# Ewenwan/ORB_SLAM2_SSD_Semantic

Measured on AMD Instinct MI355X. Metric: ORB extract+match frames/sec on 640x480 TUM RGB-D; bit-exact kp/desc, higher is better.
Workload: dtype u8

## Files before the change

orb_slam2_ssd_semantic_amd/csrc/orbfe_fast_body_u.inc:

```
    uint32_t *lflag = s_cf + wv * cf_words;
    for (int i = lane; i < cf_words; i += 64) lflag[i] = 0u;
    const OrbLane ld = lanes[(int64_t)t * 64 + lane];
    const int level = __builtin_amdgcn_readfirstlane((int)(ld.flags >> 8));
    const OrbLevel &L = plan->lv[level];
    int pitch;
    const uint8_t *src = level_ptr(fs, L, level, b, &pitch);
    uint2 *slist = skeys + (int64_t)b * plan->keys_per_frame + L.key_off;
    int32_t *scnt = scount + (b * plan->nlevels + level) * ORBFE_NK_STRIDE;
    uint32_t *cflag = cflags + (int64_t)(b * plan->nlevels + level) * cf_words;
    const int ini_th = plan->ini_th;
    uint2 *sbuf = s_buf[wv];
    int nbuf = 0;
    int st_rows = 0, st_arc = 0, st_nms = 0;
    const int key_cap = L.key_cap;
    const int ix0 = ORBFE_EDGE, iy0 = ORBFE_EDGE, ix1 = L.ix1;
    const int wcell = L.wcell, hcell = L.hcell;
    const int x = ld.x;
    const int ys = ld.ys;
    const int nrows = __builtin_amdgcn_readfirstlane((int)ld.nrows);
    const int nsteps = nrows + 7;
    const int tz = max(plan->min_th, 1);

    int ccj[4], mj[4];
    {
        const int r0 = max(x - ix0, 0);
        int c = r0 / wcell, m = r0 - c * wcell;
#pragma unroll
        for (int j = 0; j < 4; ++j) {
            if (j > 0 && x + j - ix0 >= 1) {
                ++m;
                if (m == wcell) { m = 0; ++c; }
            }
            ccj[j] = c;
            mj[j] = m;
        }
    }
    int inside = 0, lvalid = 0, rvalid = 0;
#pragma unroll
    for (int j = 0; j < 4; ++j) {
        const int xx = x + j;
        if (xx >= ix0 && xx < ix1) {
            const int m = mj[j];
            inside |= 1 << j;
            if (m != 0) lvalid |= 1 << j;
            if (m != wcell - 1 && xx + 1 < ix1) rvalid |= 1 << j;
        }
    }
    auto halves = [](int bits, int j) -> uint32_t {
        return (((bits >> j) & 1) ? 0xFFFFu : 0u) | (((bits >> (j + 1)) & 1) ? 0xFFFF0000u : 0u);
    };
    const uint32_t in01 = halves(inside, 0), in23 = halves(inside, 2);
    const uint32_t lv01 = halves(lvalid, 0), lv23 = halves(lvalid, 2);
    const uint32_t rv01 = halves(rvalid, 0), rv23 = halves(rvalid, 2);
    const bool split01 = (inside & 3) == 3 && !(lvalid & 2), split23 = (inside & 12) == 12 && !(lvalid & 8);
    const bool wave_split = orb_ballot(split01 || split23) != 0ull;
    const bool out_lane = !(ld.flags & 1) && inside != 0;
    const unsigned long long bout = orb_ballot(out_lane);
    uint32_t ordx[4];
    {
        const uint32_t row_part = (uint32_t)(((ys - iy0) / hcell) * L.ncc) << 12;
#pragma unroll
        for (int j = 0; j < 4; ++j) ordx[j] = row_part + (((uint32_t)ccj[j] << 12) | (uint32_t)mj[j]);
    }
    int rmod = 0;
    uint32_t ordy = 0u;
    const uint32_t ord_wrap = ((uint32_t)L.ncc << 12) - ((uint32_t)hcell << 6);
    const uint32_t tzz = (uint32_t)tz * 0x00010001u;
    const uint32_t resp0 = (uint32_t)(tz - 1);
    const uint32_t key00 = (uint32_t)(x - ORBFE_MINB) + ((uint32_t)(ys - 7 - ORBFE_MINB) << 12);

    uint32_t R[8][FM_NE], Raw[2][3];
    uint32_t S01[8], S23[8];
#pragma unroll
    for (int k = 0; k < 8; ++k) {
        S01[k] = S23[k] = 0u;
#pragma unroll
        for (int i = 0; i < FM_NE; ++i) R[k][i] = 0u;
    }
    const __amdgpu_buffer_rsrc_t rsrc = __builtin_amdgcn_make_buffer_rsrc((void *)src, 0, -1, 0x00020000);
    const int voff = (ys - 3) * pitch + x - 4;
    typedef uint32_t fmu_v3 __attribute__((ext_vector_type(3)));
    auto fetch = [&](int s, uint32_t (&dst3)[3]) {
        const fmu_v3 w = __builtin_amdgcn_raw_buffer_load_b96(rsrc, voff, s * pitch, 0);
        dst3[0] = w.x;
        dst3[1] = w.y;
        dst3[2] = w.z;
    };
    fetch(0, Raw[0]);

    for (int s0 = 0; s0 < nsteps; s0 += 8) {
#pragma unroll
        for (int k = 0; k < 8; ++k) {
            const int s = s0 + k;
            if (s >= nsteps) break;
            const bool have_row = s < nrows + 6;
            fetch(s + 1, Raw[(k + 1) % 2]);
            fast_unpack_row(Raw[k % 2], R[k]);
            if (s < 6) continue;
            if (have_row) {
                const uint32_t(&rm3)[FM_NE] = R[(k + 2) % 8];
                const uint32_t(&rm2)[FM_NE] = R[(k + 3) % 8];
                const uint32_t(&rm1)[FM_NE] = R[(k + 4) % 8];
                const uint32_t(&r0)[FM_NE] = R[(k + 5) % 8];
                const uint32_t(&rp1)[FM_NE] = R[(k + 6) % 8];
                const uint32_t(&rp2)[FM_NE] = R[(k + 7) % 8];
                const uint32_t(&rp3)[FM_NE] = R[k];
                bool arcs = true;
                if (SPARSE) {
                    const uint32_t p = (fast_compass_pair<0>(rm3, r0, rp3, tzz) & in01) |
                                       (fast_compass_pair<2>(rm3, r0, rp3, tzz) & in23);
                    arcs = orb_ballot(p != 0u) != 0ull;
#ifdef ORBFE_DEVELOPER
                    if (plan->dbg == 60) arcs = false;
#endif
                    if (fstat) { st_rows++; st_arc += arcs ? 0 : 1; }
                }
                if (arcs) {
                    S01[k] = fast_strength_pair<0>(rm3, rm2, rm1, r0, rp1, rp2, rp3, tzz) & in01;
                    S23[k] = fast_strength_pair<2>(rm3, rm2, rm1, r0, rp1, rp2, rp3, tzz) & in23;
                } else {
                    S01[k] = S23[k] = 0u;
                }
            }
            if (s < 7) continue;
            const int ku = (k + 6) % 8, km = (k + 7) % 8;
            const bool up_ok = rmod != 0;
            const bool dn_ok = rmod != hcell - 1 && have_row;
            const uint32_t ord_row = ordy;
            {
                const bool wrap = rmod == hcell - 1;
                rmod = wrap ? 0 : rmod + 1;
                ordy += wrap ? 64u + ord_wrap : 64u;
            }
            if (SPARSE) {
                if (orb_ballot((S01[km] | S23[km]) != 0u) == 0ull) {
                    if (fstat) st_nms++;
                    continue;
                }
            }
            const uint32_t u01 = up_ok ? S01[ku] : 0u, u23 = up_ok ? S23[ku] : 0u;
            const uint32_t d01 = dn_ok ? S01[k] : 0u, d23 = dn_ok ? S23[k] : 0u;
            const uint32_t m01 = S01[km], m23 = S23[km];
            const uint32_t v01 = pk_max_u16(u01, d01), v23 = pk_max_u16(u23, d23);
            const uint32_t c01 = pk_max_u16(v01, m01), c23 = pk_max_u16(v23, m23);
            const uint32_t cL = (uint32_t)__builtin_amdgcn_update_dpp(0, (int)c23, 0x138, 0xF, 0xF, true);
            const uint32_t cR = (uint32_t)__builtin_amdgcn_update_dpp(0, (int)c01, 0x130, 0xF, 0xF, true);
            const uint32_t l01 = __builtin_amdgcn_alignbit(c01, cL, 16) & lv01;
            const uint32_t x12 = __builtin_amdgcn_alignbit(c23, c01, 16);
            const uint32_t r23 = __builtin_amdgcn_alignbit(cR, c23, 16) & rv23;
            const uint32_t n01 = pk_max3(l01, x12 & rv01, v01);
            const uint32_t n23 = pk_max3(x12 & lv23, r23, v23);
            const uint32_t g01 = pk_subsat_u16(m01, n01), g23 = pk_subsat_u16(m23, n23);
            const unsigned long long b01 = orb_ballot(g01 != 0u) & bout, b23 = orb_ballot(g23 != 0u) & bout;
            const bool has01 = out_lane && g01 != 0u, has23 = out_lane && g23 != 0u;
            if (b01 | b23) {
                const uint32_t keyrow = key00 + ((uint32_t)s << 12);
                const int p01 = __popcll(b01);
                if (has01) {
                    const bool hi = g01 > 0xFFFFu;
                    const uint32_t a = hi ? m01 >> 16 : m01 & 0xFFFFu;
                    sbuf[nbuf + lanes_below(b01)] = make_uint2(keyrow + (hi ? 1u : 0u) + ((a + resp0) << 24),
                                                               ord_row + (hi ? ordx[1] : ordx[0]));
                }
                if (has23) {
                    const bool hi = g23 > 0xFFFFu;
                    const uint32_t a = hi ? m23 >> 16 : m23 & 0xFFFFu;
                    sbuf[nbuf + p01 + lanes_below(b23)] = make_uint2(keyrow + (hi ? 3u : 2u) + ((a + resp0) << 24),
                                                                     ord_row + (hi ? ordx[3] : ordx[2]));
                }
                nbuf += p01 + __popcll(b23);
                if (wave_split) {
                    const uint32_t gs = split01 ? g01 : (split23 ? g23 : 0u);
                    const bool dbl = out_lane && (gs & 0xFFFFu) != 0u && gs > 0xFFFFu;
                    const unsigned long long bd = orb_ballot(dbl);
                    if (bd) {
                        if (dbl) {
                            const uint32_t a = (split23 ? m23 : m01) & 0xFFFFu;
                            sbuf[nbuf + lanes_below(bd)] = make_uint2(keyrow + (split23 ? 2u : 0u) + ((a + resp0) << 24),
                                                                      ord_row + (split23 ? ordx[2] : ordx[0]));
                        }
                        nbuf += __popcll(bd);
                    }
                }
                if (nbuf > FM_BUF - FM_ROW_MAX) {
                    fm_flush(slist, scnt, sbuf, nbuf, key_cap, lane, lflag, ini_th);
                    nbuf = 0;
                }
            }
        }
    }
    if (nbuf > 0) fm_flush(slist, scnt, sbuf, nbuf, key_cap, lane, lflag, ini_th);
    __builtin_amdgcn_fence(__ATOMIC_ACQ_REL, "workgroup");
    for (int i = lane; i < cf_words; i += 64) {
        const uint32_t v = lflag[i];
        if (v) atomicOr(&cflag[i], v);
    }
    if (SPARSE && fstat && lane == 0) {
        atomicAdd(&fstat[0], (unsigned long long)st_rows);
        atomicAdd(&fstat[1], (unsigned long long)st_arc);
        atomicAdd(&fstat[2], (unsigned long long)st_nms);
    }
```

orb_slam2_ssd_semantic_amd/csrc/orbfe_kernels.hip:

```cpp
#include <stdio.h>
#include <stdlib.h>
#include <algorithm>

#include "orbfe_common.h"
#include "orbfe_kernels.h"
#include "orbfe_pattern.inc"

__constant__ signed char c_pattern[1024];
__constant__ int c_umax[16];

hipError_t orbk_upload_moment_weights(const int *umax16);

hipError_t orbk_upload_constants(const int *umax16)
{
    hipError_t e = hipMemcpyToSymbol(HIP_SYMBOL(c_pattern), orbfe_pattern31_host, 1024);
    if (e != hipSuccess) return e;
    e = hipMemcpyToSymbol(HIP_SYMBOL(c_umax), umax16, 16 * sizeof(int));
    if (e != hipSuccess) return e;
    return orbk_upload_moment_weights(umax16);
}

typedef _Float16 orb_h2 __attribute__((ext_vector_type(2)));
typedef short orb_s2 __attribute__((ext_vector_type(2)));
typedef unsigned short orb_u2 __attribute__((ext_vector_type(2)));
// ... 316 lines not shown
            uint32_t Hs[4];
            hsum(raw[(k + 1) % 4], Hs);
            const bool emit = lane_ok && d < yend && (int)(short)cur.y + 1 == r0 + s;
            const uint32_t b0 = cur.x & 0xFFFFu, b1 = cur.x >> 16;
            uint32_t pa[4], pb[4];
#pragma unroll
            for (int j = 0; j < 4; ++j) {
                pa[j] = __umul24(b0, Hp[j]);
                pb[j] = __umul24(b1, Hs[j]) + 0x20000u;
            }
            uint32_t t01, t23;
            asm("v_add_u32_sdwa %0, %1, %2 dst_sel:DWORD dst_unused:UNUSED_PAD src0_sel:WORD_1 src1_sel:WORD_1" : "=v"(t01) : "v"(pa[0]), "v"(pb[0]));
            asm("v_add_u32_sdwa %0, %1, %2 dst_sel:WORD_1 dst_unused:UNUSED_PRESERVE src0_sel:WORD_1 src1_sel:WORD_1" : "+v"(t01) : "v"(pa[1]), "v"(pb[1]));
            asm("v_add_u32_sdwa %0, %1, %2 dst_sel:DWORD dst_unused:UNUSED_PAD src0_sel:WORD_1 src1_sel:WORD_1" : "=v"(t23) : "v"(pa[2]), "v"(pb[2]));
            asm("v_add_u32_sdwa %0, %1, %2 dst_sel:WORD_1 dst_unused:UNUSED_PRESERVE src0_sel:WORD_1 src1_sel:WORD_1" : "+v"(t23) : "v"(pa[3]), "v"(pb[3]));
            const uint32_t q01 = __builtin_bit_cast(uint32_t, __builtin_bit_cast(orb_u2, t01) >> (orb_u2)(2));
            const uint32_t q23 = __builtin_bit_cast(uint32_t, __builtin_bit_cast(orb_u2, t23) >> (orb_u2)(2));
            if (emit) {
                *park = __builtin_amdgcn_perm(q23, q01, 0x06040200u);
                park += GX;
                d += 1;
            }
            cur = s_yt[min(d, yend) - by0];
#pragma unroll
            for (int j = 0; j < 4; ++j) Hp[j] = Hs[j];
        }
    }
    if (lane_ok && g0 + cg < ncol4) {
        uint32_t oofs = __umul24((uint32_t)y0, (uint32_t)a.dpitch) + (uint32_t)dx0;
        const int nrows = yend - y0;
        for (int i0 = 0; i0 < a.rb; i0 += 8) {
            uint32_t v[8];
#pragma unroll
            for (int i = 0; i < 8; ++i) v[i] = s_tile[(yl0 + min(i0 + i, a.rb - 1)) * GX + cg];
#pragma unroll
            for (int i = 0; i < 8; ++i)
                if (i0 + i < nrows) *(uint32_t *)(dst + (oofs + (uint32_t)(i0 + i) * (uint32_t)a.dpitch)) = v[i];
        }
    }
    __syncthreads();
    const int cx0 = p.cxs[tx], cx1 = p.cxs[tx + 1], cy0 = p.cys[ty], cy1 = p.cys[ty + 1];
    if (cx1 <= cx0 || cy1 <= cy0) return;
    const int gq0 = cx0 >> 2, ngc = ((cx1 - 1) >> 2) - gq0 + 1;
    const int nch = max(1, 256 / ngc);
    const int gi = (int)threadIdx.x % ngc, chn = (int)threadIdx.x / ngc;
    if (chn >= nch) return;
    const int nrowsC = cy1 - cy0, per = (nrowsC + nch - 1) / nch;
    const int ya = cy0 + chn * per, yb = min(ya + per, cy1);
    const uint8_t *T = (const uint8_t *)s_tile;
    const int tpitch = GX * 4, bx0 = g0 * 4;
    const int colmax = min(GX * 4, W - bx0) - 1, rowmax = min(trows, H - by0) - 1;
    uint8_t *dstC = p.dstC + (int64_t)b * a.dst_fstride;
    const int xg = (gq0 + gi) * 4;
    int c0i[4], c1i[4];
    uint32_t cc0[4], cc1[4];
    bool ok[4];
#pragma unroll
    for (int j = 0; j < 4; ++j) {
        const int x2 = xg + j;
        ok[j] = x2 >= cx0 && x2 < cx1;
        const OrbTab tt = p.xtabC[min(x2, p.cw - 1)];
        c0i[j] = min(max((int)tt.s - bx0, 0), colmax);
        c1i[j] = min(c0i[j] + 1, colmax);
        cc0[j] = (uint32_t)(uint16_t)tt.c0;
        cc1[j] = (uint32_t)(uint16_t)tt.c1;
    }
    const bool full = ok[0] && ok[1] && ok[2] && ok[3];
    OrbTab tyn = p.ytabC[min(ya, p.ch - 1)];
    for (int y2 = ya; y2 < yb; ++y2) {
        const OrbTab ty_ = tyn;
        tyn = p.ytabC[min(y2 + 1, p.ch - 1)];
        const int rr0 = (int)ty_.s - by0, rr1 = min(rr0 + 1, rowmax);
        const uint32_t b0 = (uint32_t)(uint16_t)ty_.c0, b1 = (uint32_t)(uint16_t)ty_.c1;
        const uint8_t *R0 = T + rr0 * tpitch, *R1 = T + rr1 * tpitch;
        uint32_t px[4];
#pragma unroll
        for (int j = 0; j < 4; ++j) {
            const uint32_t H0 = (R0[c0i[j]] * cc0[j] + R0[c1i[j]] * cc1[j]) >> 4, H1 = (R1[c0i[j]] * cc0[j] + R1[c1i[j]] * cc1[j]) >> 4;
            px[j] = ((((b0 * H0) >> 16) + ((b1 * H1) >> 16) + 2u) >> 2) & 0xFFu;
        }
        uint8_t *o = dstC + (__umul24((uint32_t)y2, (uint32_t)p.cpitch) + (uint32_t)xg);
        if (full) {
            *(uint32_t *)o = px[0] | (px[1] << 8) | (px[2] << 16) | (px[3] << 24);
        } else {
#pragma unroll
            for (int j = 0; j < 4; ++j)
                if (ok[j]) o[j] = (uint8_t)px[j];
        }
    }
}
#endif

__device__ __forceinline__ unsigned long long orb_ballot(bool p) { return __builtin_amdgcn_ballot_w64(p); }
__device__ __forceinline__ int min3i(int a, int b, int c) { return min(min(a, b), c); }
__device__ __forceinline__ int max3i(int a, int b, int c) { return max(max(a, b), c); }



__device__ __forceinline__ uint32_t pk_min3(uint32_t a, uint32_t b, uint32_t c)
{
    const orb_h2 x = __builtin_bit_cast(orb_h2, a), y = __builtin_bit_cast(orb_h2, b), z = __builtin_bit_cast(orb_h2, c);
    return __builtin_bit_cast(uint32_t, __builtin_elementwise_minimum(__builtin_elementwise_minimum(x, y), z));
}
__device__ __forceinline__ uint32_t pk_max3(uint32_t a, uint32_t b, uint32_t c)
{
    const orb_h2 x = __builtin_bit_cast(orb_h2, a), y = __builtin_bit_cast(orb_h2, b), z = __builtin_bit_cast(orb_h2, c);
    return __builtin_bit_cast(uint32_t, __builtin_elementwise_maximum(__builtin_elementwise_maximum(x, y), z));
}
__device__ __forceinline__ uint32_t pk_sub_i16(uint32_t a, uint32_t b)
{
    return __builtin_bit_cast(uint32_t, __builtin_bit_cast(orb_s2, a) - __builtin_bit_cast(orb_s2, b));
}
__device__ __forceinline__ uint32_t pk_max_i16(uint32_t a, uint32_t b)
{
    return __builtin_bit_cast(uint32_t, __builtin_elementwise_max(__builtin_bit_cast(orb_s2, a), __builtin_bit_cast(orb_s2, b)));
}
__device__ __forceinline__ uint32_t pk_sub_u16(uint32_t a, uint32_t b)
{
    return __builtin_bit_cast(uint32_t, __builtin_bit_cast(orb_u2, a) - __builtin_bit_cast(orb_u2, b));
}
__device__ __forceinline__ uint32_t pk_max_u16(uint32_t a, uint32_t b)
{
    return __builtin_bit_cast(uint32_t, __builtin_elementwise_max(__builtin_bit_cast(orb_u2, a), __builtin_bit_cast(orb_u2, b)));
}
__device__ __forceinline__ uint32_t pk_min_u16(uint32_t a, uint32_t b)
{
    return __builtin_bit_cast(uint32_t, __builtin_elementwise_min(__builtin_bit_cast(orb_u2, a), __builtin_bit_cast(orb_u2, b)));
}
__device__ __forceinline__ uint32_t pk_subsat_u16(uint32_t a, uint32_t b)
{
    return __builtin_bit_cast(uint32_t, __builtin_elementwise_sub_sat(__builtin_bit_cast(orb_u2, a), __builtin_bit_cast(orb_u2, b)));
}

template <int IDX>
__device__ __forceinline__ uint32_t rowpair(const uint32_t (&w)[3])
{
    static_assert(IDX >= 0 && IDX < 11, "window pair");
    if ((IDX & 3) < 3)
        return __builtin_amdgcn_perm(0u, w[IDX >> 2], 0x0c000c00u | ((uint32_t)((IDX & 3) + 1) << 16) | (uint32_t)(IDX & 3));
    return __builtin_amdgcn_perm(w[(IDX >> 2) + 1 > 2 ? 2 : (IDX >> 2) + 1], w[IDX >> 2], 0x0c040c03u);
}

#define FM_NE 9
__device__ __forceinline__ void fast_unpack_row(const uint32_t (&w)[3], uint32_t (&e)[FM_NE])
{
    e[0] = rowpair<1>(w);
    e[1] = rowpair<2>(w);
    e[2] = rowpair<3>(w);
    e[3] = rowpair<4>(w);
    e[4] = rowpair<5>(w);
    e[5] = rowpair<6>(w);
    e[6] = rowpair<7>(w);
    e[7] = rowpair<8>(w);
    e[8] = rowpair<9>(w);
}

template <int J>
__device__ __forceinline__ uint32_t fast_strength_pair(const uint32_t (&rm3)[FM_NE], const uint32_t (&rm2)[FM_NE],
                                                       const uint32_t (&rm1)[FM_NE], const uint32_t (&r0)[FM_NE],
                                                       const uint32_t (&rp1)[FM_NE], const uint32_t (&rp2)[FM_NE],
                                                       const uint32_t (&rp3)[FM_NE], uint32_t t)
{
    uint32_t c[16];
    c[0] = rp3[3 + J];
    c[1] = rp3[4 + J];
    c[2] = rp2[5 + J];
    c[3] = rp1[6 + J];
    c[4] = r0[6 + J];
    c[5] = rm1[6 + J];
    c[6] = rm2[5 + J];
    c[7] = rm3[4 + J];
    c[8] = rm3[3 + J];
    c[9] = rm3[2 + J];
    c[10] = rm2[1 + J];
    c[11] = rm1[0 + J];
    c[12] = r0[0 + J];
    c[13] = rp1[0 + J];
    c[14] = rp2[1 + J];
    c[15] = rp3[2 + J];
    const uint32_t v = r0[3 + J];
    uint32_t P[8], Q[8], ex[8], en[8];
#pragma unroll
    for (int i = 0; i < 8; ++i) {
        P[i] = pk_min_u16(c[2 * i + 1], c[(2 * i + 2) & 15]);
        Q[i] = pk_max_u16(c[2 * i + 1], c[(2 * i + 2) & 15]);
        ex[i] = pk_max_u16(c[2 * i], c[(2 * i + 9) & 15]);
        en[i] = pk_min_u16(c[2 * i], c[(2 * i + 9) & 15]);
    }
    uint32_t Wb[8], Wd[8];
#pragma unroll
    for (int i = 0; i < 8; i += 2) {
        const uint32_t ab = pk_min3(P[i], P[(i + 1) & 7], P[(i + 2) & 7]);
        const uint32_t ad = pk_max3(Q[i], Q[(i + 1) & 7], Q[(i + 2) & 7]);
        Wb[i] = pk_min3(ab, P[(i + 3) & 7], ex[i]);
        Wd[i] = pk_max3(ad, Q[(i + 3) & 7], en[i]);
        Wb[(i + 7) & 7] = pk_min3(P[(i + 7) & 7], ab, ex[(i + 7) & 7]);
        Wd[(i + 7) & 7] = pk_max3(Q[(i + 7) & 7], ad, en[(i + 7) & 7]);
    }
    const uint32_t maxmin = pk_max_u16(pk_max3(pk_max3(pk_max3(Wb[0], Wb[1], Wb[2]), Wb[3], Wb[4]), Wb[5], Wb[6]), Wb[7]);
    const uint32_t minmax = pk_min_u16(pk_min3(pk_min3(pk_min3(Wd[0], Wd[1], Wd[2]), Wd[3], Wd[4]), Wd[5], Wd[6]), Wd[7]);
    const uint32_t m = pk_max3(pk_subsat_u16(v, minmax), pk_subsat_u16(maxmin, v), t);
    return pk_sub_u16(m, t);
}

template <int J>
__device__ __forceinline__ uint32_t fast_compass_pair(const uint32_t (&rm3)[FM_NE], const uint32_t (&r0)[FM_NE],
                                                      const uint32_t (&rp3)[FM_NE], uint32_t t)
{
    const uint32_t c0 = rp3[3 + J], c8 = rm3[3 + J];
    const uint32_t c4 = r0[6 + J], c12 = r0[0 + J];
    const uint32_t v = r0[3 + J];
    const uint32_t mb = pk_min_u16(pk_max_u16(c0, c8), pk_max_u16(c4, c12));
    const uint32_t md = pk_max_u16(pk_min_u16(c0, c8), pk_min_u16(c4, c12));
    return pk_subsat_u16(pk_max_u16(pk_subsat_u16(mb, v), pk_subsat_u16(v, md)), t);
}

__device__ __forceinline__ uint32_t fast_strength_from(const uint32_t (&c)[16], uint32_t v, uint32_t t)
{
    uint32_t P[8], Q[8], ex[8], en[8];
#pragma unroll
    for (int i = 0; i < 8; ++i) {
        P[i] = pk_min_u16(c[2 * i + 1], c[(2 * i + 2) & 15]);
        Q[i] = pk_max_u16(c[2 * i + 1], c[(2 * i + 2) & 15]);
        ex[i] = pk_max_u16(c[2 * i], c[(2 * i + 9) & 15]);
        en[i] = pk_min_u16(c[2 * i], c[(2 * i + 9) & 15]);
    }
    uint32_t Wb[8], Wd[8];
#pragma unroll
    for (int i = 0; i < 8; i += 2) {
        const uint32_t ab = pk_min3(P[i], P[(i + 1) & 7], P[(i + 2) & 7]);
        const uint32_t ad = pk_max3(Q[i], Q[(i + 1) & 7], Q[(i + 2) & 7]);
        Wb[i] = pk_min3(ab, P[(i + 3) & 7], ex[i]);
        Wd[i] = pk_max3(ad, Q[(i + 3) & 7], en[i]);
        Wb[(i + 7) & 7] = pk_min3(P[(i + 7) & 7], ab, ex[(i + 7) & 7]);
        Wd[(i + 7) & 7] = pk_max3(Q[(i + 7) & 7], ad, en[(i + 7) & 7]);
    }
    const uint32_t maxmin = pk_max_u16(pk_max3(pk_max3(pk_max3(Wb[0], Wb[1], Wb[2]), Wb[3], Wb[4]), Wb[5], Wb[6]), Wb[7]);
    const uint32_t minmax = pk_min_u16(pk_min3(pk_min3(pk_min3(Wd[0], Wd[1], Wd[2]), Wd[3], Wd[4]), Wd[5], Wd[6]), Wd[7]);
    const uint32_t m = pk_max3(pk_subsat_u16(v, minmax), pk_subsat_u16(maxmin, v), t);
    return pk_sub_u16(m, t);
}

__device__ __forceinline__ int lanes_below(unsigned long long m)
{
    return __builtin_amdgcn_mbcnt_hi((uint32_t)(m >> 32), __builtin_amdgcn_mbcnt_lo((uint32_t)m, 0));
}

#define FM_BUF 384
#define FM_ROW_MAX 140

__device__ __forceinline__ void fm_flush(uint2 *slist, int32_t *scnt, const uint2 *sbuf, int nbuf, int key_cap, int lane,
                                         uint32_t *lflag, int ini)
{
    int base = 0;
    if (lane == 0) base = atomicAdd(scnt, nbuf);
    base = __shfl(base, 0, 64);
    for (int i = lane; i < nbuf; i += 64) {
        const uint2 e = sbuf[i];
        if (base + i < key_cap) slist[base + i] = e;
        if (orb_key_r(e.x) >= ini) {
            const uint32_t cell = e.y >> 12;
            atomicOr(&lflag[cell >> 5], 1u << (cell & 31));
        }
    }
}

#if defined(FM_WAVES_PER_EU)
#define FM_OCC __attribute__((amdgpu_waves_per_eu(FM_WAVES_PER_EU, FM_WAVES_PER_EU)))
#else
#define FM_OCC
#endif
#define FM_SHARED_DECLS                                                                                             \
    __shared__ uint2 s_buf[4][FM_BUF];                                                                              \
    extern __shared__ uint32_t s_cf[];
#ifdef FM_LDS_CONSTS
#define FM_LDS_DECLS                                                             \
    __shared__ uint4 s_lcm[4][64];                   \
    __shared__ uint2 s_lcr[4][64];                               \
    __shared__ uint4 s_lco[4][64];
#else
#define FM_LDS_DECLS
#endif

template <int SPARSE>
__global__ __launch_bounds__(256) FM_OCC void k_fast_map(const OrbPlan *__restrict__ plan, FrameSrc fs,
                                                  const OrbLane *__restrict__ lanes, int nwaves,
                                                  uint2 *__restrict__ skeys,
                                                  int32_t *__restrict__ scount,
                                                  uint32_t *__restrict__ cflags,
                                                  int32_t cf_words,
                                                  unsigned long long *__restrict__ fstat)
{
    FM_SHARED_DECLS
    FM_LDS_DECLS
    int b = blockIdx.y, bx = blockIdx.x;
    xcd_frame_remap(bx, b);
    const int lane = threadIdx.x & 63;
    const int wv = threadIdx.x >> 6;
    const int t = bx * (blockDim.x >> 6) + wv;
    if (t >= nwaves) return;
#include "orbfe_fast_body.inc"
}

template <int SPARSE>
__global__ __launch_bounds__(256) FM_OCC void k_fast_map_u(const OrbPlan *__restrict__ plan, FrameSrc fs,
                                                    const OrbLane *__restrict__ lanes, int nwaves,
                                                    uint2 *__restrict__ skeys, int32_t *__restrict__ scount,
                                                    uint32_t *__restrict__ cflags, int32_t cf_words,
                                                    unsigned long long *__restrict__ fstat)
{
    FM_SHARED_DECLS
    int b = blockIdx.y, bx = blockIdx.x;
    xcd_frame_remap(bx, b);
    const int lane = threadIdx.x & 63;
    const int wv = threadIdx.x >> 6;
    const int t = bx * (blockDim.x >> 6) + wv;
    if (t >= nwaves) return;
#include "orbfe_fast_body_u.inc"
}

#define FC_QCAP 128
#ifndef FC_LAG
#define FC_LAG 3
#endif
#define FC_PN (6 + FC_LAG)
#define FC_PW 66
#define FC_SEAMS 16
#define FC_BUF (128 + FC_SEAMS)
#ifndef FC_OCC
#define FC_OCC
#endif
static_assert(FC_LAG >= 1 && FC_LAG <= 3, "the strength-row ring (srow / snap, 4 slots) is re-used by the front half of step s + 4: the back half of step s must have read it, i.e. lag <= 3");
static_assert(FC_PN >= 6 + FC_LAG && FC_PN >= 7, "pixel ring: the first row of an item parked at step s is overwritten at step s - 6 + FC_PN");
__device__ __forceinline__ uint32_t fast_compass_from(uint32_t c0, uint32_t c8, uint32_t c4, uint32_t c12, uint32_t v, uint32_t t)
{
    const uint32_t mb = pk_min_u16(pk_max_u16(c0, c8), pk_max_u16(c4, c12));
    const uint32_t md = pk_max_u16(pk_min_u16(c0, c8), pk_min_u16(c4, c12));
    return pk_subsat_u16(pk_max_u16(pk_subsat_u16(mb, v), pk_subsat_u16(v, md)), t);
}
__global__ __launch_bounds__(256) FC_OCC void k_fast_map_c(const OrbPlan *__restrict__ plan, FrameSrc fs,
                                                    const OrbLane *__restrict__ lanes, int nwaves,
                                                    uint2 *__restrict__ skeys, int32_t *__restrict__ scount,
                                                    uint32_t *__restrict__ cflags, int32_t cf_words,
                                                    unsigned long long *__restrict__ fstat)
{
    __shared__ uint32_t s_pix[4][2 * FC_PN * FC_PW];
#ifdef FC_EXTRA_LDS
    __shared__ uint32_t s_fcpad[FC_EXTRA_LDS / 4];
    if (nwaves < 0) s_fcpad[threadIdx.x] = 1u;
    if (nwaves < -1) scount[0] = (int32_t)s_fcpad[threadIdx.x ^ 1];
#endif
    __shared__ uint32_t s_q[4][FC_QCAP];
    __shared__ uint32_t s_srow[4][4 * 64];
    __shared__ uint2 s_buf[4][FC_BUF];
    extern __shared__ uint32_t s_cf[];
    int b = blockIdx.y, bx = blockIdx.x;
    xcd_frame_remap(bx, b);
    const int lane = threadIdx.x & 63;
    const int wv = threadIdx.x >> 6;
    const int t = bx * (blockDim.x >> 6) + wv;
    if (t >= nwaves) return;
#include "orbfe_fast_body_c.inc"
}

#ifdef ORBFE_DEVELOPER
template <int SPARSE>
__global__ __launch_bounds__(256) void k_fast_pyr(const OrbPlan *__restrict__ plan, FrameSrc fs, const OrbLane *__restrict__ lanes,
                                                  int wave_lo, int nwaves, uint2 *__restrict__ skeys, int32_t *__restrict__ scount,
                                                  uint32_t *__restrict__ cflags, int32_t cf_words,
                                                  unsigned long long *__restrict__ fstat, PyrArgs pa, int npyr, int spread)
{
    FM_SHARED_DECLS
    FM_LDS_DECLS
    int b = blockIdx.y, bx = blockIdx.x;
    xcd_frame_remap(bx, b);
    int before = min(bx, npyr);
    bool is_pyr = bx < npyr;
    if (spread) {
        const int T = (int)gridDim.x;
        before = (int)(((uint32_t)bx * (uint32_t)npyr) / (uint32_t)T);
        is_pyr = (int)(((uint32_t)(bx + 1) * (uint32_t)npyr) / (uint32_t)T) > before;
    }
    if (is_pyr) {
        const PyrArgs &a = pa;
        const uint32_t bxi = (uint32_t)before;
#include "orbfe_pyr_body.inc"
        return;
    }
    const int lane = threadIdx.x & 63;
    const int wv = threadIdx.x >> 6;
    if ((bx - before) * 4 + wv >= nwaves) return;
    const int t = wave_lo + (bx - before) * 4 + wv;
#include "orbfe_fast_body.inc"
}
#endif

#define QT_MAX 512
struct OctGroup {
    int32_t level0;
    int32_t M;
    int32_t nini;
    int32_t tw, th;
    int32_t ncells;
};
#define KNODE_MASK 0x3FFFu
#ifndef KUNROLL
#define KUNROLL 8
#endif
#define FFD 5
#define FF_PER_ROOT 1364
__host__ __device__ inline int ff_off(int d) { return ((1 << (2 * d)) - 4) / 3; }

struct QtShared {
    int M;
    int32_t *cnt0;
    uint32_t *path0;
    __device__ __forceinline__ int32_t *cnt(int g) const { return cnt0 + g * M; }
    __device__ __forceinline__ uint32_t *path(int g) const { return path0 + g * M; }
    int32_t *cc;
    int32_t *P;
    int32_t *rankOf0;
    __device__ __forceinline__ int32_t *rankOf(int g) const { return rankOf0 + g * M; }
    int32_t *acc;
    int32_t *newIdx;
    unsigned long long *skey;
    int32_t *hist;
    uint16_t *xtab;
    uint16_t *ytab;
    uint32_t *cflag;
    int32_t *misc;
    int16_t *gbox;
    __device__ __forceinline__ int16_t *box(int g, int j) const { return gbox + (g * 4 + j) * M; }
};

__host__ __device__ inline int qt_pow2(int v)
{
    int p = 2;
    while (p < v) p <<= 1;
    return p;
}

__device__ __forceinline__ void qt_carve(char *lds, char *nodes, int M, int nroots, int w, int h, int ncells, QtShared &q)
{
    char *p = nodes;
    q.skey = (unsigned long long *)p; p += (size_t)qt_pow2(M) * 8;
    q.cc = (int32_t *)p; p += (size_t)M * 16;
    q.M = M;
    q.cnt0 = (int32_t *)p; p += (size_t)M * 8;
    q.path0 = (uint32_t *)p; p += (size_t)M * 8;
    q.P = (int32_t *)p; p += (size_t)M * 4;
    q.rankOf0 = (int32_t *)p; p += (size_t)M * 8;
    q.acc = (int32_t *)p; p += (size_t)M * 4;
    q.newIdx = (int32_t *)p; p += (size_t)M * 4;
    p = nodes == lds ? p : lds;
    q.hist = (int32_t *)p; p += (size_t)nroots * FF_PER_ROOT * 4;
    q.misc = (int32_t *)p; p += 64 * 4;
    q.xtab = (uint16_t *)p; p += (size_t)((w + 1) & ~1) * 2;
    q.ytab = (uint16_t *)p; p += (size_t)((h + 1) & ~1) * 2;
    q.cflag = (uint32_t *)p;
}

size_t orbk_octree_node_bytes(int M) { return (((size_t)qt_pow2(M) * 8 + (size_t)M * (16 + 8 + 8 + 20)) + 255) & ~(size_t)255; }
static size_t octree_table_bytes(int nroots, int w, int h, int ncells)
{
    return (size_t)nroots * FF_PER_ROOT * 4 + 64 * 4 + (size_t)(((w + 1) & ~1) + ((h + 1) & ~1)) * 2 + (size_t)((ncells + 31) / 32) * 4;
}
size_t orbk_octree_lds_bytes(int M, int nroots, int w, int h, int ncells)
{
    return (size_t)qt_pow2(M) * 8 + (size_t)M * (16 + 8 + 8 + 20) + octree_table_bytes(nroots, w, h, ncells);
}

size_t orbk_octree_box_bytes(int M) { return (size_t)M * 2 * 4 * sizeof(int16_t); }

__device__ __forceinline__ int wave_min_i(int v)
{
#pragma unroll
    for (int o = 32; o > 0; o >>= 1) v = min(v, __shfl_xor(v, o, 64));
    return v;
}

__device__ __forceinline__ int bscan_inclusive(int32_t *arr, int n, int32_t *sw)
{
    const int tid = threadIdx.x, QT = blockDim.x, wid = tid >> 6, lane = tid & 63, nw = QT >> 6;
    int carry = 0;
    for (int base = 0; base < n; base += QT) {
        const int i = base + tid;
        const int v = i < n ? arr[i] : 0;
        const int incl = wave_incl_scan(v);
        if (lane == 63) sw[wid] = incl;
        __syncthreads();
        int pre = 0, tot = 0;
        for (int w = 0; w < nw; ++w) {
            const int t = sw[w];
            pre += w < wid ? t : 0;
            tot += t;
        }
        if (i < n) arr[i] = carry + pre + incl;
        carry += tot;
        __syncthreads();
    }
    return carry;
}

__device__ __forceinline__ void qt_sort_assign(const QtShared &q, int Mp, int nToExpand, int S2, int nx)
{
    const int tid = threadIdx.x, QT = blockDim.x;
    for (int kk = 2; kk <= Mp; kk <<= 1)
        for (int j = kk >> 1; j > 0; j >>= 1) {
            for (int i = tid; i < Mp; i += QT) {
                const int ixj = i ^ j;
                if (ixj > i) {
                    const unsigned long long a = q.skey[i], c2 = q.skey[ixj];
                    const bool desc = (i & kk) == 0;
                    if (desc ? (a < c2) : (a > c2)) { q.skey[i] = c2; q.skey[ixj] = a; }
                }
            }
            __syncthreads();
        }
    for (int i = tid; i < S2; i += QT) q.rankOf(nx)[i] = -1;
    __syncthreads();
    for (int r = tid; r < nToExpand; r += QT) {
        const int pos = (int)(q.skey[r] & 0xFFFFull);
        q.P[r] = pos;
        q.rankOf(nx)[pos] = r;
    }
}

__device__ __forceinline__ void bscan2_inclusive(int32_t *a, int na, int32_t *b, int nb, int32_t *sw, int &ta, int &tb)
{
    const int tid = threadIdx.x, QT = blockDim.x, wid = tid >> 6, lane = tid & 63, nw = QT >> 6;
    int ca = 0, cb = 0;
    for (int base = 0; base < max(na, nb); base += QT) {
        const int i = base + tid;
        const int va = i < na ? a[i] : 0, vb = i < nb ? b[i] : 0;
        const int ia = wave_incl_scan(va), ib = wave_incl_scan(vb);
        if (lane == 63) { sw[wid] = ia; sw[8 + wid] = ib; }
        __syncthreads();
        int pa = 0, pb = 0, sa = 0, sb = 0;
        for (int w = 0; w < nw; ++w) {
            const int x = sw[w], y = sw[8 + w];
            pa += w < wid ? x : 0;
            pb += w < wid ? y : 0;
            sa += x;
            sb += y;
        }
        if (i < na) a[i] = ca + pa + ia;
        if (i < nb) b[i] = cb + pb + ib;
        ca += sa;
        cb += sb;
        __syncthreads();
    }
    ta = ca;
    tb = cb;
}

__device__ __forceinline__ void qt_pass_bfs_hist(const QtShared &q, int N, int &S, int &m, int &cur, int &modeB, bool &finish)
{
    const int tid = threadIdx.x, QT = blockDim.x;
    const int nx = cur ^ 1;
    int32_t *sw = q.misc + 32;
    int32_t *pk = q.acc, *un = q.newIdx;
    auto quad = [&](int i) {
        const uint32_t pth = q.path(cur)[i];
        const int d = (int)((pth >> 12) & 0xFu), root = (int)(pth >> 16);
        return &q.hist[root * FF_PER_ROOT + ff_off(d + 1) + (int)((pth & 0xFFFu) << 2)];
    };
    for (int r = tid; r < m; r += QT) {
        const int32_t *c = quad(q.P[r]);
        pk[r] = ((c[0] > 0) + (c[1] > 0) + (c[2] > 0) + (c[3] > 0)) | (((c[0] > 1) + (c[1] > 1) + (c[2] > 1) + (c[3] > 1)) << 16);
    }
    for (int i = tid; i < S; i += QT) un[i] = q.rankOf(cur)[i] < 0 ? 1 : 0;
    __syncthreads();
    int tpk, nUnproc;
    bscan2_inclusive(pk, m, un, S, sw, tpk, nUnproc);
    const int totalChildren = tpk & 0xFFFF, nToExpand = tpk >> 16;
    const int S2 = totalChildren + nUnproc;
    finish = (S2 >= N) || (S2 == S);
    const int modeB2 = (!finish && (S2 + 3 * nToExpand > N)) ? 1 : 0;
    int Mp = 2;
    if (modeB2) {
        while (Mp < nToExpand) Mp <<= 1;
        for (int i = tid; i < Mp; i += QT) q.skey[i] = 0ull;
        __syncthreads();
    }
    for (int i = tid; i < S; i += QT) {
        const int r = q.rankOf(cur)[i];
        const uint32_t pth = q.path(cur)[i];
        if (r >= 0) {
            const int inc = pk[r];
            const int32_t *c = quad(i);
            const int c0 = c[0], c1 = c[1], c2 = c[2], c3 = c[3];
            const int cn[4] = {c0, c1, c2, c3};
            int pos = totalChildren - (inc & 0xFFFF);
            int mr = nToExpand - (inc >> 16);
            int seq = (inc >> 16) - ((c0 > 1) + (c1 > 1) + (c2 > 1) + (c3 > 1));
            int seqq[4];
#pragma unroll
            for (int qd = 0; qd < 4; ++qd) { seqq[qd] = seq; seq += cn[qd] > 1 ? 1 : 0; }
            const uint32_t cpath = (pth & 0xFFFF0000u) | ((((pth >> 12) & 0xFu) + 1u) << 12) | ((pth & 0xFFFu) << 2);
#pragma unroll
            for (int qd = 3; qd >= 0; --qd) {
                if (cn[qd] > 0) {
                    q.cnt(nx)[pos] = cn[qd];
                    q.path(nx)[pos] = cpath | (uint32_t)qd;
                    if (cn[qd] > 1) {
                        if (modeB2) {
                            q.skey[seqq[qd]] = ((unsigned long long)(uint32_t)cn[qd] << 32) |
                                               ((unsigned long long)(uint32_t)(seqq[qd] + 1) << 16) | (unsigned long long)pos;
                        } else {
                            q.P[mr] = pos;
                            q.rankOf(nx)[pos] = mr;
                        }
                        ++mr;
                    } else if (!modeB2) {
// ... 1541 lines not shown
```

Before: 306,500.

## Batch FAST keypoint emission per 8-row block using LDS score ring

Rather than ballot-compacting and writing keypoints to the shared buffer after every row's non-max suppression, each lane now packs its per-row survivor bits into a 32-bit pending mask. It stores the 8-bit scores in a per-wave LDS ring, and once per 8-row block it drains the mask with a ctz/ballot loop to emit the entries. This takes the per-row ballots, popcounts and divergent stores out of the inner loop and drops the special split-lane double-emit path. The cost is extra LDS for the ring, a smaller staging buffer, and more complex reconstruction of the key and order fields, including the cell wrap offset.

```diff
diff --git a/orb_slam2_ssd_semantic_amd/csrc/orbfe_fast_body_u.inc b/orb_slam2_ssd_semantic_amd/csrc/orbfe_fast_body_u.inc
--- a/orb_slam2_ssd_semantic_amd/csrc/orbfe_fast_body_u.inc
+++ b/orb_slam2_ssd_semantic_amd/csrc/orbfe_fast_body_u.inc
@@ -10,7 +10,14 @@
     uint32_t *cflag = cflags + (int64_t)(b * plan->nlevels + level) * cf_words;
     const int ini_th = plan->ini_th;
     uint2 *sbuf = s_buf[wv];
+    uint32_t *aring = s_ring[wv] + lane;
     int nbuf = 0;
+    uint32_t pend = 0u;
+    uint32_t ordblk = 0u;
+    int wk = 8;
+#ifdef ORBFE_DEVELOPER
+    const bool dbg_noemit = plan->dbg == 61;
+#endif
     int st_rows = 0, st_arc = 0, st_nms = 0;
     const int key_cap = L.key_cap;
     const int ix0 = ORBFE_EDGE, iy0 = ORBFE_EDGE, ix1 = L.ix1;
@@ -52,10 +59,7 @@
     const uint32_t in01 = halves(inside, 0), in23 = halves(inside, 2);
     const uint32_t lv01 = halves(lvalid, 0), lv23 = halves(lvalid, 2);
     const uint32_t rv01 = halves(rvalid, 0), rv23 = halves(rvalid, 2);
-    const bool split01 = (inside & 3) == 3 && !(lvalid & 2), split23 = (inside & 12) == 12 && !(lvalid & 8);
-    const bool wave_split = orb_ballot(split01 || split23) != 0ull;
     const bool out_lane = !(ld.flags & 1) && inside != 0;
-    const unsigned long long bout = orb_ballot(out_lane);
     uint32_t ordx[4];
     {
         const uint32_t row_part = (uint32_t)(((ys - iy0) / hcell) * L.ncc) << 12;
@@ -126,9 +130,13 @@
             const int ku = (k + 6) % 8, km = (k + 7) % 8;
             const bool up_ok = rmod != 0;
             const bool dn_ok = rmod != hcell - 1 && have_row;
-            const uint32_t ord_row = ordy;
+            if (k == 0 || (k == 7 && s0 == 0)) {
+                ordblk = ordy - 64u * (uint32_t)k;
+                wk = 8;
+            }
             {
                 const bool wrap = rmod == hcell - 1;
+                if (wrap) wk = k;
                 rmod = wrap ? 0 : rmod + 1;
                 ordy += wrap ? 64u + ord_wrap : 64u;
             }
@@ -151,44 +159,44 @@
             const uint32_t n01 = pk_max3(l01, x12 & rv01, v01);
             const uint32_t n23 = pk_max3(x12 & lv23, r23, v23);
             const uint32_t g01 = pk_subsat_u16(m01, n01), g23 = pk_subsat_u16(m23, n23);
-            const unsigned long long b01 = orb_ballot(g01 != 0u) & bout, b23 = orb_ballot(g23 != 0u) & bout;
-            const bool has01 = out_lane && g01 != 0u, has23 = out_lane && g23 != 0u;
-            if (b01 | b23) {
-                const uint32_t keyrow = key00 + ((uint32_t)s << 12);
-                const int p01 = __popcll(b01);
-                if (has01) {
-                    const bool hi = g01 > 0xFFFFu;
-                    const uint32_t a = hi ? m01 >> 16 : m01 & 0xFFFFu;
-                    sbuf[nbuf + lanes_below(b01)] = make_uint2(keyrow + (hi ? 1u : 0u) + ((a + resp0) << 24),
-                                                               ord_row + (hi ? ordx[1] : ordx[0]));
-                }
-                if (has23) {
-                    const bool hi = g23 > 0xFFFFu;
-                    const uint32_t a = hi ? m23 >> 16 : m23 & 0xFFFFu;
-                    sbuf[nbuf + p01 + lanes_below(b23)] = make_uint2(keyrow + (hi ? 3u : 2u) + ((a + resp0) << 24),
-                                                                     ord_row + (hi ? ordx[3] : ordx[2]));
-                }
-                nbuf += p01 + __popcll(b23);
-                if (wave_split) {
-                    const uint32_t gs = split01 ? g01 : (split23 ? g23 : 0u);
-                    const bool dbl = out_lane && (gs & 0xFFFFu) != 0u && gs > 0xFFFFu;
-                    const unsigned long long bd = orb_ballot(dbl);
-                    if (bd) {
-                        if (dbl) {
-                            const uint32_t a = (split23 ? m23 : m01) & 0xFFFFu;
-                            sbuf[nbuf + lanes_below(bd)] = make_uint2(keyrow + (split23 ? 2u : 0u) + ((a + resp0) << 24),
-                                                                      ord_row + (split23 ? ordx[2] : ordx[0]));
-                        }
-                        nbuf += __popcll(bd);
-                    }
-                }
-                if (nbuf > FM_BUF - FM_ROW_MAX) {
+            const uint32_t f01 = g01 + 0x00FF00FFu, f23 = g23 + 0x00FF00FFu;
+            pend |= __builtin_amdgcn_perm(f23, f01, 0x07050301u) << k;
+            aring[k * 64] = __builtin_amdgcn_perm(m23, m01, 0x06040200u);
+        }
+        {
+            uint32_t pw = out_lane ? pend : 0u;
+            pend = 0u;
+            const uint32_t keyblk = key00 + ((uint32_t)s0 << 12);
+            unsigned long long bp = orb_ballot(pw != 0u);
+            while (bp) {
+#ifdef ORBFE_DEVELOPER
+                if (dbg_noemit) {
+                    nbuf += __popcll(bp);
+                    if (nbuf > FMU_BUF - 64) nbuf = 0;
+                    break;
+                }
+#endif
+                if (nbuf > FMU_BUF - 64) {
                     fm_flush(slist, scnt, sbuf, nbuf, key_cap, lane, lflag, ini_th);
                     nbuf = 0;
                 }
-            }
-        }
-    }
+                if (pw != 0u) {
+                    const uint32_t i = (uint32_t)__builtin_ctz(pw);
+                    pw &= pw - 1u;
+                    const uint32_t kk = i & 7u, p = i >> 3;
+                    const uint32_t a = (aring[kk * 64] >> (i & 24u)) & 0xFFu;
+                    const uint32_t ox = p == 0u ? ordx[0] : (p == 1u ? ordx[1] : (p == 2u ? ordx[2] : ordx[3]));
+                    sbuf[nbuf + lanes_below(bp)] = make_uint2(keyblk + (kk << 12) + p + ((a + resp0) << 24),
+                                                              ordblk + (kk << 6) + ((int)kk > wk ? ord_wrap : 0u) + ox);
+                }
+                nbuf += __popcll(bp);
+                bp = orb_ballot(pw != 0u);
+            }
+        }
+    }
+#ifdef ORBFE_DEVELOPER
+    if (dbg_noemit) nbuf = 0;
+#endif
     if (nbuf > 0) fm_flush(slist, scnt, sbuf, nbuf, key_cap, lane, lflag, ini_th);
     __builtin_amdgcn_fence(__ATOMIC_ACQ_REL, "workgroup");
     for (int i = lane; i < cf_words; i += 64) {
diff --git a/orb_slam2_ssd_semantic_amd/csrc/orbfe_kernels.hip b/orb_slam2_ssd_semantic_amd/csrc/orbfe_kernels.hip
--- a/orb_slam2_ssd_semantic_amd/csrc/orbfe_kernels.hip
+++ b/orb_slam2_ssd_semantic_amd/csrc/orbfe_kernels.hip
@@ -642,6 +642,7 @@
 #include "orbfe_fast_body.inc"
 }
 
+#define FMU_BUF 128
 template <int SPARSE>
 __global__ __launch_bounds__(256) FM_OCC void k_fast_map_u(const OrbPlan *__restrict__ plan, FrameSrc fs,
                                                     const OrbLane *__restrict__ lanes, int nwaves,
@@ -649,7 +650,9 @@
                                                     uint32_t *__restrict__ cflags, int32_t cf_words,
                                                     unsigned long long *__restrict__ fstat)
 {
-    FM_SHARED_DECLS
+    __shared__ uint2 s_buf[4][FMU_BUF];
+    __shared__ uint32_t s_ring[4][8 * 64];
+    extern __shared__ uint32_t s_cf[];
     int b = blockIdx.y, bx = blockIdx.x;
     xcd_frame_remap(bx, b);
     const int lane = threadIdx.x & 63;
```

Measured after the change: 308,100 (median of 6 runs). Within noise of the previous version (+0.5%).
